# NCKempke/PIPS-IPMpp

Measured on AMD Instinct MI355X. Metric: KKT factor+solve per IPM iter/sec, N-block arrowhead LP, higher is better.
Workload: dtype f64; 1 GPU; 64 blocks x 10000 vars (5000 eq rows, rho=0.001), Schur dim 2000, 64 blocks/GPU [BASELINE configs[1]]; deterministic=False, family=random, root=dense LDL^T, sparse_head=multifrontal (k_front), solves_per_unit=4, collective=none, nnzL_per_gpu=649118456

## Files before the change

### pips-ipmpp_amd/csrc/engine.hip

```cpp
#include <hip/hip_runtime.h>

#include <algorithm>
#include <cstdlib>
#include <cstring>
#include <map>
#include <memory>
#include <mutex>
#include <thread>
#include <vector>

#include "common.h"
#include "devmem.h"
#include "layout.h"
#include "kernels.hip.h"
#include "rootkernel.hip.h"
#include "tailkernel.hip.h"
#include "pips_hip.h"

namespace pips {

static thread_local std::string g_last_error;
void set_last_error(const std::string& msg) { g_last_error = msg; }
std::atomic<long long> g_host_waits{0};
struct WaitSite { std::atomic<const char*> file{nullptr}; std::atomic<int> line{0}; std::atomic<long long> n{0}; };
// ... 82 lines not shown
         end(upd_diag[j]);
         begin(upd[j]);
         const int P = (pair2 > 1 && panel == 0 && split_diag && diag_ahead) ? pair2 : 1;
         const int g = j / P * P, q = j - g;
         if (j > p0 && split_diag && diag_ahead)
            for (int b = 0; b < nblk; ++b)
               if (blks[b].ntc > j + 1) {
                  const int k0 = std::max(p0, fst(b, j + 1)), lo = q > 0 ? std::max(k0, g) : k0;
                  if (lo < j) all.push_back({b, j + 1, j + 1, lo | (j << 16)});
               }
         if (P > 1 && q == 0 && j > p0)
            for (int b = 0; b < nblk; ++b)
               for (int d = j + 2; d <= j + P && d < blks[b].ntc; ++d) {
                  const int k0 = std::max(p0, fst(b, d));
                  if (k0 < j) all.push_back({b, d, d, k0 | (j << 16)});
               }
         if (j > p0)
            for (int b = 0; b < nblk; ++b)
               if (blks[b].ntc > j)
                  for (int ti = split_diag ? j + 1 : j; ti < blks[b].ntr; ++ti) {
                     if (j >= fst(b, ti)) {
                        const int k0 = std::max({p0, fst(b, ti), fst(b, j)}), lo = q > 0 ? std::max(k0, g) : k0;
                        if (lo < j) all.push_back({b, ti, j, lo | (j << 16)});
                     }
                     if (P > 1 && q == 0)
                        for (int c = j + 1; c < j + P && c < blks[b].ntc && c < ti; ++c)
                           if (c >= fst(b, ti)) {
                              const int k0 = std::max({p0, fst(b, ti), fst(b, c)});
                              if (k0 < j) all.push_back({b, ti, c, k0 | (j << 16)});
                           }
                  }
         end(upd[j]);
         begin(diag[j]);
         for (int b = 0; b < nblk; ++b)
            if (blks[b].ntc > j) all.push_back({b, j, j, 0});
         end(diag[j]);
         begin(trsm[j]);
         for (int b = 0; b < nblk; ++b)
            if (blks[b].ntc > j)
               for (int ti = j + 1; ti < blks[b].ntr; ++ti)
                  if (j >= fst(b, ti)) all.push_back({b, ti, j, 0});
         end(trsm[j]);
         begin(fwd[j]);
         for (int b = 0; b < nblk; ++b)
            if (blks[b].ntc > j)
               for (int ti = j; ti < blks[b].ntc; ++ti)
                  if (ti == j || (j >= 1 && j - 1 >= fst(b, ti))) all.push_back({b, ti, j, 0});
         end(fwd[j]);
         begin(bwd[j]);
         for (int b = 0; b < nblk; ++b)
            if (blks[b].ntc > j)
               for (int tj = 0; tj <= j; ++tj)
                  if (tj == j || (j + 1 < blks[b].ntc && tj >= fst(b, j + 1))) all.push_back({b, tj, j, 0});
         end(bwd[j]);
         if (panel > 0 && (j + 1) % panel == 0) {
            begin(trail_next[j]);
            if (lookahead)
               for (int b = 0; b < nblk; ++b)
                  if (j + 1 < blks[b].ntc)
                     for (int ti = j + 1; ti < blks[b].ntr; ++ti) all.push_back({b, ti, j + 1, p0 | ((j + 1) << 16)});
            end(trail_next[j]);
            begin(trail[j]);
            for (int b = 0; b < nblk; ++b)
               for (int tj = j + (lookahead ? 2 : 1); tj < blks[b].ntc; ++tj)
                  for (int ti = tj; ti < blks[b].ntr; ++ti) all.push_back({b, ti, tj, p0 | ((j + 1) << 16)});
            end(trail[j]);
         }
      }
      begin(schur);
      for (int b = 0; b < nblk; ++b)
         if (blks[b].ntc > 0 && blks[b].nb > 0) {
            const int nt = blks[b].nb_pad / TILE;
            for (int ti = 0; ti < nt; ++ti)
               for (int tj = 0; tj <= ti; ++tj) all.push_back({b, ti, tj, 0});
         }
      end(schur);
      h_tasks = all;
      return d_tasks.upload(all);
   }
};

struct SweepRt {
   DevBuf<TileTask> d_tasks;
   int n_tasks = 0;
   DevBuf<int> d_ints;
   long long n_flags = 0;
   DevBuf<long long> d_flag_off, d_tfirst_off;
   DevBuf<int> d_tfirst;
   int epoch = 0;
   bool enabled = false;
   long long poll_limit = SWEEP_POLL_LIMIT;
   int take_error(const char* who) {
      if (!d_ints) return PIPS_OK;
      int w = 0;
      HIP_TRY(hipMemcpy(&w, d_ints + 2 * SWEEP_NRHS_MAX, sizeof(int), hipMemcpyDeviceToHost));
      if (!w) return PIPS_OK;
      HIP_TRY(hipMemset(d_ints + 2 * SWEEP_NRHS_MAX, 0, sizeof(int)));
      PIPS_FAIL(PIPS_ERR_HIP, "%s: a single-launch solve sweep gave up waiting for a piece of the solution after %lld polls (its output is NaN); "
                              "another process holding the device for seconds can cause that - PIPS_HIP_SWEEP_LAUNCHES=1 selects the launch-per-column sweeps",
                who, poll_limit);
   }
   int build(const std::vector<BlkDesc>& blks, const std::vector<const std::vector<int>*>* first) {
      *this = SweepRt();
      if (const char* pl = getenv("PIPS_HIP_SWEEP_POLL_LIMIT")) poll_limit = atoll(pl);
      const int nblk = (int)blks.size();
      int ntc_max = 0;
      for (auto& b : blks) ntc_max = std::max(ntc_max, b.ntc);
      std::vector<TileTask> tasks;
      for (int i = 0; i < ntc_max; ++i)
         for (int b = 0; b < nblk; ++b)
            if (i < blks[b].ntc) tasks.push_back({b, i, 0, 0});
      n_tasks = (int)tasks.size();
      std::vector<long long> foff(nblk), tfoff(nblk);
      std::vector<int> tf;
      long long nf = 0;
      for (int b = 0; b < nblk; ++b) {
         foff[b] = nf;
         nf += blks[b].ntc;
         tfoff[b] = (long long)tf.size();
         if (first)
            for (int i = 0; i < blks[b].ntr; ++i) tf.push_back(i < blks[b].ntc ? std::min(i, (*(*first)[b])[i]) : (*(*first)[b])[i]);
      }
      int rc;
      if ((rc = d_tasks.upload(tasks))) return rc;
      if ((rc = d_flag_off.upload(foff))) return rc;
      if (first) {
         if ((rc = d_tfirst.upload(tf))) return rc;
         if ((rc = d_tfirst_off.upload(tfoff))) return rc;
      }
      n_flags = std::max<long long>(nf, 1);
      const size_t ints = (size_t)(2 * SWEEP_NRHS_MAX + 2 + n_flags * SWEEP_NRHS_MAX);
      PIPS_TRY(d_ints.alloc_zero(ints));
      epoch = 0;
      enabled = n_tasks > 0 && !getenv("PIPS_HIP_SWEEP_LAUNCHES");
      return PIPS_OK;
   }
   SweepArgs args(long long xw_stride, hipStream_t st) {
      int* ep = d_ints + 2 * SWEEP_NRHS_MAX + 1;
      hipLaunchKernelGGL(k_sweep_bump, dim3(1), dim3(1), 0, st, ep);
      return SweepArgs{d_tasks, n_tasks, d_ints, d_ints + 2 * SWEEP_NRHS_MAX + 2, d_flag_off, d_tfirst, d_tfirst_off, ep,
                       d_ints + 2 * SWEEP_NRHS_MAX, n_flags, xw_stride, poll_limit};
   }
};

struct PhaseTimer {
   bool on = false;
   struct Rec { hipEvent_t a, b; int phase; };
   std::vector<Rec> recs;
   std::vector<hipEvent_t> pool;
   size_t used = 0;
   static constexpr int NPHASE = 16;
   double ms[NPHASE] = {0};
   long long cnt[NPHASE] = {0};
   hipEvent_t get() {
      if (used == pool.size()) {
         hipEvent_t e;
         (void)hipEventCreate(&e);
         pool.push_back(e);
      }
      return pool[used++];
   }
   void reset() { recs.clear(); used = 0; }
   void begin(hipStream_t s, int phase) {
      if (!on) return;
      Rec r{get(), get(), phase};
      (void)hipEventRecord(r.a, s);
      recs.push_back(r);
   }
   void end(hipStream_t s) {
      if (!on) return;
      (void)hipEventRecord(recs.back().b, s);
   }
   int begin_i(hipStream_t s, int phase) {
      if (!on) return -1;
      begin(s, phase);
      return (int)recs.size() - 1;
   }
   void end_i(int idx, hipStream_t s) {
      if (on && idx >= 0) (void)hipEventRecord(recs[idx].b, s);
   }
   void collect() {
      for (int i = 0; i < NPHASE; ++i) { ms[i] = 0; cnt[i] = 0; }
      for (auto& r : recs) {
         float t = 0;
         if (hipEventElapsedTime(&t, r.a, r.b) == hipSuccess) { ms[r.phase] += t; ++cnt[r.phase]; }
      }
   }
   ~PhaseTimer() { for (auto e : pool) (void)hipEventDestroy(e); }
};

struct TailSingle {
   TailLdlArgs args{};
   DevBuf<TileTask> d_tasks;
   DevBuf<int> d_flags, d_flags_init, d_ctl;
   DevBuf<long long> d_flag_off;
   long long n_flags = 0;
   int n_tasks = 0, n_blocks = 0;
   int build(const TailPlan& p, const std::vector<BlkDesc>& blks, hipStream_t stream) {
      *this = TailSingle();
      const int nblk = (int)blks.size();
      n_blocks = nblk;
      std::vector<long long> foff(nblk + 1, 0);
      for (int b = 0; b < nblk; ++b) foff[b + 1] = foff[b] + (long long)blks[b].ntr * blks[b].ntc + blks[b].ntr + blks[b].ntc;
      n_flags = foff[nblk];
      std::vector<int> init((size_t)std::max<long long>(n_flags, 1), 0);
      for (int b = 0; b < nblk; ++b)
         for (int ti = 0; ti < blks[b].ntr; ++ti)
            for (int tj = 0; tj < blks[b].ntc; ++tj) init[foff[b] + (long long)ti * blks[b].ntc + tj] = -1;
      std::vector<TileTask> order;
      auto take = [&](const TaskList& l, int kind) {
         for (long long q = l.off; q < l.off + l.cnt; ++q) {
            TileTask t = p.h_tasks[q];
            if (t.blk < 0) continue;
            if (kind == ROOT_UPD) {
               int& pr = init[foff[t.blk] + (long long)t.ti * blks[t.blk].ntc + t.tj];
               if (pr < 0) pr = t.pad & 0xffff;
            } else
               t.pad = 0;
            t.blk |= kind << 24;
            order.push_back(t);
         }
      };
      std::vector<int> row_first((size_t)std::max<long long>(n_flags, 1), 1 << 20);
// ... 171 lines not shown
         hipLaunchKernelGGL(k_tile_diag, dim3(p.diag[j].cnt), dim3(256), 0, c.side, p.d_tasks + p.diag[j].off,
                            c.d_blks, c.d_arena, c.d_dtail, c.d_winv, c.d_psign, c.d_psign_off, c.d_inertia, c.d_pref);
         HIP_TRY(hipEventRecord(c.ev_rest, c.side));
      } else if (p.upd_diag[j].cnt > 0) {
         gemm_diag_tiles(p.upd_diag[j], c.stream);
      }
      if (p.upd[j].cnt > 0) {
         if (c.timer) c.timer->begin(c.stream, 2);
         gemm0(p.upd[j], c.stream);
         if (c.timer) c.timer->end(c.stream);
      }
      if (ahead) {
         HIP_TRY(hipStreamWaitEvent(c.stream, c.ev_rest, 0));
      } else {
         if (c.timer) c.timer->begin(c.stream, 3);
         if (c.bunch_kaufman)
            hipLaunchKernelGGL(k_tile_diag_bk, dim3(p.diag[j].cnt), dim3(256), 0, c.stream, p.d_tasks + p.diag[j].off, c.d_blks, c.d_arena, c.d_dtail,
                               c.d_winv, c.d_inertia, c.d_pert_cnt, c.d_pert_list, c.bk_orig, c.bk_orig_ld, c.bk_orig_rowmajor, c.d_bk_perm, c.bk_isolate);
         else
         hipLaunchKernelGGL(k_tile_diag, dim3(p.diag[j].cnt), dim3(256), 0, c.stream, p.d_tasks + p.diag[j].off,
                            c.d_blks, c.d_arena, c.d_dtail, c.d_winv, c.d_psign, c.d_psign_off, c.d_inertia, c.d_pref);
         if (c.timer) c.timer->end(c.stream);
      }
      if (p.trsm[j].cnt > 0) {
         if (c.timer) c.timer->begin(c.stream, 4);
         hipLaunchKernelGGL(k_tile_gemm<1>, dim3((p.trsm[j].cnt + 7) / 8 * 8), dim3(512), 0, c.stream, p.d_tasks + p.trsm[j].off, p.trsm[j].cnt,
                            c.d_blks, c.d_arena, c.d_dtail, c.d_winv, c.d_bmap, (double*)nullptr, 0, (const int*)nullptr, c.d_uarena);
         if (c.timer) c.timer->end(c.stream);
         if (c.bunch_kaufman && c.is_root && c.d_pert_cnt)
            hipLaunchKernelGGL(k_bk_growth, dim3(TILE), dim3(256), 0, c.stream, c.d_blks, c.d_arena, j, 1e8, c.d_pert_cnt, c.d_pert_list);
      }
      if (p.trail_next[j].cnt > 0 || p.trail[j].cnt > 0) {
         if ((rc = main_writes(j + 1))) return rc;
         const bool split = c.side && p.trail[j].cnt > 0;
         if (split) {
            HIP_TRY(hipEventRecord(c.ev_panel, c.stream));
            HIP_TRY(hipStreamWaitEvent(c.side, c.ev_panel, 0));
            gemm0(p.trail[j], c.side);
            HIP_TRY(hipEventRecord(c.ev_rest, c.side));
            side_busy = true;
            side_from = j + 2;
         }
         if (c.timer) c.timer->begin(c.stream, 2);
         if (p.trail_next[j].cnt > 0) gemm0(p.trail_next[j], c.stream);
         if (!split && p.trail[j].cnt > 0) gemm0(p.trail[j], c.stream);
         if (c.timer) c.timer->end(c.stream);
      }
   }
   if ((rc = main_writes(1 << 30))) return rc;
   if (SC && c.det_rounds) {
      if (c.timer) c.timer->begin(c.stream, 5);
      for (const TaskList& l : *c.det_rounds)
         if (l.cnt > 0)
            hipLaunchKernelGGL(k_tile_gemm<2>, dim3((l.cnt + 7) / 8 * 8), dim3(512), 0, c.stream, c.d_det_tasks + l.off, l.cnt, c.d_blks, c.d_arena,
                               c.d_dtail, c.d_winv, c.d_bmap, SC, ldSC, c.d_sctab, c.d_uarena, c.d_gbuf, c.gstride, c.d_blk_group);
      if (!c.det_reduce_later) reduce_det_groups(c, SC, ldSC);
      if (c.timer) c.timer->end(c.stream);
   } else if (SC && c.sc_groups && !c.d_sctab) {
      if (c.timer) c.timer->begin(c.stream, 5);
      for (size_t g = 0; g < c.sc_groups->size(); ++g) {
         const TaskList& l = (*c.sc_groups)[g];
         if (l.cnt > 0)
            hipLaunchKernelGGL(k_tile_gemm<2>, dim3((l.cnt + 7) / 8 * 8), dim3(512), 0, c.stream, c.d_sc_tasks + l.off, l.cnt, c.d_blks, c.d_arena,
                               c.d_dtail, c.d_winv, c.d_bmap, SC, ldSC, c.d_sctab, c.d_uarena);
         HIP_TRY(hipEventRecord((*c.ev_sc)[g], c.stream));
      }
      if (c.timer) c.timer->end(c.stream);
   } else if (SC && p.schur.cnt > 0 && c.d_ctr_pool && !c.d_sctab && *c.ctr_cursor < GEMM_CTR_SLOTS) {
      if (c.timer) c.timer->begin(c.stream, 5);
      const int wgs = ((p.schur.cnt + 7) / 8 * 8) / 8 * 9;
      hipLaunchKernelGGL(k_tile_gemm_bal<2>, dim3((wgs + 7) / 8 * 8), dim3(512), 0, c.stream, p.d_tasks + p.schur.off, p.schur.cnt, c.d_blks,
                         c.d_arena, c.d_dtail, c.d_winv, c.d_bmap, SC, ldSC, c.d_sctab, c.d_uarena, c.d_ctr_pool + 8 * (*c.ctr_cursor)++);
      if (c.timer) c.timer->end(c.stream);
   } else if (SC && p.schur.cnt > 0) {
      if (c.timer) c.timer->begin(c.stream, 5);
      hipLaunchKernelGGL(k_tile_gemm<2>, dim3((p.schur.cnt + 7) / 8 * 8), dim3(512), 0, c.stream, p.d_tasks + p.schur.off, p.schur.cnt, c.d_blks,
                         c.d_arena, c.d_dtail, c.d_winv, c.d_bmap, SC, ldSC, c.d_sctab, c.d_uarena);
      if (c.timer) c.timer->end(c.stream);
   }
   HIP_TRY(hipGetLastError());
   return PIPS_OK;
}

static int tail_fwd(const TailCtx& c, double* xw, int nrhs = 1, long long xw_stride = 0) {
   const TailPlan& p = *c.plan;
   if (c.sweep && c.sweep->enabled && nrhs <= SWEEP_NRHS_MAX) {
      hipLaunchKernelGGL(k_tail_rows_fwd, dim3(c.sweep->n_tasks, nrhs), dim3(256), 0, c.stream, c.sweep->args(xw_stride, c.stream), c.d_blks, c.d_arena, c.d_dtail,
                         c.d_winv, xw);
      HIP_TRY(hipGetLastError());
      return PIPS_OK;
   }
   for (int j = 0; j < p.ntc_max; ++j)
      if (p.fwd[j].cnt > 0)
         hipLaunchKernelGGL(k_tail_fwd, dim3(p.fwd[j].cnt, nrhs), dim3(256), 0, c.stream, p.d_tasks + p.fwd[j].off, c.d_blks,
                            c.d_arena, c.d_dtail, c.d_winv, xw, j, xw_stride);
   HIP_TRY(hipGetLastError());
   return PIPS_OK;
}

static int tail_bwd(const TailCtx& c, double* xw, int nrhs = 1, long long xw_stride = 0, int border = 0) {
   const TailPlan& p = *c.plan;
   if (p.ntc_max == 0) return PIPS_OK;
   if (border && !(c.sweep && c.sweep->enabled)) PIPS_FAIL(PIPS_ERR_STATE, "border-backward sweep needs the single-launch tail sweeps");
   if (c.sweep && c.sweep->enabled && nrhs <= SWEEP_NRHS_MAX) {
      hipLaunchKernelGGL(k_tail_rows_bwd, dim3(c.sweep->n_tasks, nrhs), dim3(256), 0, c.stream, c.sweep->args(xw_stride, c.stream), c.d_blks, c.d_arena, c.d_dtail,
                         c.d_winv, xw, border);
      HIP_TRY(hipGetLastError());
      return PIPS_OK;
   }
   for (int i = p.ntc_max - 1; i >= 0; --i)
      if (p.bwd[i].cnt > 0)
         hipLaunchKernelGGL(k_tail_bwd, dim3(p.bwd[i].cnt, nrhs), dim3(256), 0, c.stream, p.d_tasks + p.bwd[i].off, c.d_blks,
                            c.d_arena, c.d_dtail, c.d_winv, xw, i, xw_stride);
   HIP_TRY(hipGetLastError());
   return PIPS_OK;
}


struct AnalyzeKnobs : LayoutKnobs {
   long long tail_poll_limit = 0;
   int tail_diag_blocked = 1;
};
struct Engine;
static void read_layout_knobs(const Engine* e, AnalyzeOptions& opt, AnalyzeKnobs& knobs);

struct EngineAnalysis {
   DevBuf<double> d_norms;
   PinnedBuf<double> h_norms;
   DevBuf<int> d_frowptr, d_fcol, d_fsrc;
   DevBuf<long long> d_flong;
   DevBuf<int> d_sctab;
   DevBuf<int> d_schur_cols, d_schur_slot;
   DevBuf<int> d_kb_rec;
   DevBuf<long long> d_kb_off;
   DevBuf<int> d_kb_list;
   DevBuf<int> d_kb_tail;
   DevBuf<double> d_mfU;
   DevBuf<double> d_mfLV;
   DevBuf<int> d_roots, d_root_off;
   DevBuf<BbBatch> d_bb_batches;
   DevBuf<BbMeta> d_bb_meta;
   DevBuf<int> d_bb_off, d_bb_pos;
   DevBuf<double> d_bb_out;
   DevBuf<int> d_bb_round_blk;
   DevBuf<int> d_round_blk;
   DevBuf<int> d_mfint;
   DevBuf<long long> d_mfdbg;
   DevBuf<int> d_spine, d_spine_off;
   TailPlan plan;
   SweepRt sweep;
   TailSingle tsingle;
   DevBuf<double> d_uarena;
   DevBuf<double> d_arena, d_kval, d_bval, d_winv, d_dtail, d_xw, d_rhs, d_res, d_stage, d_pref;
   DevBuf<long long> d_kdst, d_bdst, d_kdiag, d_kptr, d_psign_off, d_perm_off, d_rowbase, d_bt_xoff;
   DevBuf<SnDesc> d_sns;
   DevBuf<BlkDesc> d_blks;
   DevBuf<int> d_lf_rows, d_lf_ptr, d_lf_src, d_lf_pos;
   DevBuf<double> d_lf_val;
   DevBuf<LeafDesc> d_leafdesc;
   DevBuf<int> d_lb_list;
   DevBuf<int> d_rowidx, d_upd, d_sncol, d_bmap, d_perm, d_inertia, d_nprimal;
   DevBuf<int> d_br_rowptr, d_br_sc, d_br_src;
   DevBuf<int> d_krowptr, d_kcolidx, d_bt_rowptr, d_bt_colidx, d_bt_rowsc;
   DevBuf<signed char> d_psign;
   struct GatherList {
      long long n_targets = 0, n_slots = 0;
      DevBuf<long long> d_tgt, d_off, d_slots;
   };
   struct SlotEntry { long long target, slot; };
   DevBuf<double> d_slot_val, d_vslot_val;
// ... 1141 lines not shown
      const bool need_amax = refine_mode == 1 && h_amax.empty();
      if (need_amax) {
         tmp.resize(nblk);
         HIP_TRY(hipMemcpyAsync(tmp.data(), d_blks, (size_t)nblk * sizeof(BlkDesc), hipMemcpyDeviceToHost, stream));
      }
      HIP_TRY(hipStreamSynchronize(stream));
      if (need_amax) {
         h_amax.resize(nblk);
         for (int b = 0; b < nblk; ++b) h_amax[b] = tmp[b].repl_abs / (repl_rel > 0 ? repl_rel : 1.0);
      }
      double worst = 0.0;
      for (int b = 0; b < nblk; ++b) {
         const double den = refine_mode == 1 ? h_amax[b] * h_norms[2 * nblk + b] + h_norms[nblk + b] : h_norms[nblk + b];
         if (den > 0.0) { const double q = h_norms[b] / den; if (!(q <= worst)) worst = q; }
      }
      *worst_out = worst;
      last_refine_measure = worst;
      return PIPS_OK;
   }

   int fetch_inertia() {
      if (inertia_in_flight && h_inertia_pin) {
         HIP_TRY(hipEventSynchronize(ev_inertia));
         std::copy(h_inertia_pin.get(), h_inertia_pin + h_inertia.size(), h_inertia.begin());
         inertia_in_flight = false;
         inertia_on_host = true;
         if (tail_single && h_inertia_pin[3 * nblk]) {
            h_inertia_pin[3 * nblk] = 0;
            int fi[6] = {0, 0, 0, 0, 0, 0};
            (void)hipMemcpy(fi, tsingle.d_ctl + 10, sizeof(fi), hipMemcpyDeviceToHost);
            HIP_TRY(hipMemsetAsync(tsingle.d_ctl + 9, 0, 7 * sizeof(int), stream));
            PIPS_FAIL(PIPS_ERR_HIP, "the single-launch factorisation of the dense tails (PIPS_HIP_TAIL_SINGLE) gave up waiting for a tile after %lld polls - first: task "
                                    "kind %d on tile (%d, %d) of block %d; its factors are unusable.  Another process holding the device for seconds can cause that",
                      tsingle.args.poll_limit, fi[1], fi[2], fi[3], fi[5] - 1);
         }
         return PIPS_OK;
      }
      if (inertia_on_host) return PIPS_OK;
      HIP_TRY(hipMemcpyAsync(h_inertia.data(), d_inertia, h_inertia.size() * sizeof(int), hipMemcpyDeviceToHost, stream));
      HIP_TRY(hipStreamSynchronize(stream));
      return PIPS_OK;
   }

   long long aug_passes = 0;
   int perturbed_cache = -1;
   int perturbed_leaf_pivots(int* out) {
      if (perturbed_cache < 0) {
         int rc = fetch_inertia();
         if (rc) return rc;
         int z = 0;
         for (int b = 0; b < nblk; ++b) z += h_inertia[3 * b + 2];
         perturbed_cache = z;
      }
      *out = perturbed_cache;
      return PIPS_OK;
   }
   int forward_augmented(const double* b_dev, double* red) {
      if (!factored) PIPS_FAIL(PIPS_ERR_STATE, "solve called before factor");
      HIP_TRY(hipSetDevice(device));
      timer.begin(stream, 7);
      hipLaunchKernelGGL(k_border_fill, dim3(8, nblk), dim3(256), 0, stream, d_blks, d_bmap, (const double*)nullptr, d_xw, 0.0);
      hipLaunchKernelGGL(k_permute_in, dim3(64, nblk, 1), dim3(256), 0, stream, d_blks, d_perm, d_perm_off, b_dev, 0LL, d_xw, 0LL);
      timer.end(stream);
      timer.begin(stream, 8);
      for (const LevelRange& L : levels) {
         if (L.simple_cnt > 0 && lf_rows > 0)
            hipLaunchKernelGGL(k_leaf_fwd_gather, dim3((unsigned)((lf_rows + 255) / 256), 1), dim3(256), 0, stream, d_lf_rows, d_lf_ptr, d_lf_src, d_lf_val, d_xw,
                               0LL, (int)lf_rows);
         else if (L.simple_cnt > 0)
            hipLaunchKernelGGL(k_head_solve_simple, dim3((L.simple_cnt + 255) / 256, 1), dim3(256), 0, stream, d_sns, L.simple_begin, L.simple_cnt, d_blks,
                               d_rowidx, d_arena, d_xw, 0LL, 0);
         if (L.simple_cnt > 0 && n_lb > 0)
            hipLaunchKernelGGL(k_leaf_border, dim3((n_lb + 255) / 256), dim3(256), 0, stream, d_lb_list, n_lb, d_sns, d_blks, d_rowidx, d_arena, d_xw, 0);
         const int begin = L.small_cnt > 0 ? L.small_begin : L.large_begin;
         const int cnt = L.small_cnt + L.large_cnt;
         if (cnt > 0)
            hipLaunchKernelGGL(head_wcap <= 16 ? k_head_fwd_chain<16> : k_head_fwd_chain<HEAD_WMAX>, dim3(cnt, 1), dim3(64), 0, stream, d_sns, begin, d_blks,
                               d_rowidx, d_arena, d_xw, 0LL, 1);
      }
      timer.end(stream);
      timer.begin(stream, 9);
      TailCtx c = ctx();
      c.timer = nullptr;
      int rc = tail_fwd(c, d_xw);
      if (rc) return rc;
      if (nb_pad_max > 0)
         hipLaunchKernelGGL(k_tail_border_fwd, dim3(nb_pad_max / TILE, nblk), dim3(256), 0, stream, d_blks, d_arena, d_dtail, d_xw);
      hipLaunchKernelGGL(k_border_collect, dim3(8, nblk), dim3(256), 0, stream, d_blks, d_bmap, d_xw, red);
      timer.end(stream);
      ++aug_passes;
      HIP_TRY(hipGetLastError());
      return PIPS_OK;
   }
   int forward_augmented_det(const double* b_dev) {
      if (!factored) PIPS_FAIL(PIPS_ERR_STATE, "solve called before factor");
      if (!det_aug_ready || !head_slots) PIPS_FAIL(PIPS_ERR_STATE, "forward_augmented_det: not prepared");
      HIP_TRY(hipSetDevice(device));
      timer.begin(stream, 7);
      hipLaunchKernelGGL(k_border_fill, dim3(8, nblk), dim3(256), 0, stream, d_blks, d_bmap, (const double*)nullptr, d_xw, 0.0);
      hipLaunchKernelGGL(k_permute_in, dim3(64, nblk, 1), dim3(256), 0, stream, d_blks, d_perm, d_perm_off, b_dev, 0LL, d_xw, 0LL);
      timer.end(stream);
      timer.begin(stream, 8);
      const ScatterCtx sxv{2, nullptr, d_vslot_val, d_xw, nullptr};
      for (size_t li = 0; li < levels.size(); ++li) {
         const LevelRange& L = levels[li];
         gather(gv_levels[li], d_vslot_val, d_xw);
         if (L.simple_cnt > 0 && lf_rows > 0)
            hipLaunchKernelGGL(k_leaf_fwd_gather, dim3((unsigned)((lf_rows + 255) / 256), 1), dim3(256), 0, stream, d_lf_rows, d_lf_ptr, d_lf_src, d_lf_val, d_xw,
                               0LL, (int)lf_rows);
         else if (L.simple_cnt > 0)
            hipLaunchKernelGGL(k_head_solve_simple, dim3((L.simple_cnt + 255) / 256, 1), dim3(256), 0, stream, d_sns, L.simple_begin, L.simple_cnt, d_blks,
                               d_rowidx, d_arena, d_xw, 0LL, 0, sxv);
         const int begin = L.small_cnt > 0 ? L.small_begin : L.large_begin;
         const int cnt = L.small_cnt + L.large_cnt;
         if (cnt > 0) hipLaunchKernelGGL(k_head_fwd, dim3(cnt, 1), dim3(64), 0, stream, d_sns, begin, d_blks, d_rowidx, d_arena, d_xw, 0LL, sxv);
      }
      gather(gv_tail, d_vslot_val, d_xw);
      hipLaunchKernelGGL(k_border_rowdot_det, dim3(grid_for(n_bg_ent, 256, 1 << 20)), dim3(256), 0, stream, n_bg_ent, d_bg_ent, d_arena, d_xw, d_bg_val);
      hipLaunchKernelGGL(k_border_gather_det, dim3((unsigned)((n_bg_targets + 3) / 4)), dim3(256), 0, stream, n_bg_targets, d_bg_ptr, d_bg_idx, d_bg_slot, d_bg_val, d_xw);
      timer.end(stream);
      timer.begin(stream, 9);
      TailCtx c = ctx();
      c.timer = nullptr;
      int rc = tail_fwd(c, d_xw);
      if (rc) return rc;
      if (nb_pad_max > 0)
         hipLaunchKernelGGL(k_tail_border_fwd, dim3(nb_pad_max / TILE, nblk), dim3(256), 0, stream, d_blks, d_arena, d_dtail, d_xw);
      timer.end(stream);
      ++aug_passes;
      HIP_TRY(hipGetLastError());
      return PIPS_OK;
   }
   int backward_augmented(const double* x0_dev, double* out_dev) {
      if (!factored) PIPS_FAIL(PIPS_ERR_STATE, "solve called before factor");
      HIP_TRY(hipSetDevice(device));
      timer.begin(stream, 10);
      hipLaunchKernelGGL(k_border_fill, dim3(8, nblk), dim3(256), 0, stream, d_blks, d_bmap, x0_dev, d_xw, 1.0);
      TailCtx c = ctx();
      c.timer = nullptr;
      int rc = tail_bwd(c, d_xw, 1, 0, 1);
      if (rc) return rc;
      for (int l = (int)levels.size() - 1; l >= 0; --l) {
         const LevelRange& L = levels[l];
         const int begin = L.small_cnt > 0 ? L.small_begin : L.large_begin;
         const int cnt = L.small_cnt + L.large_cnt;
         if (cnt > 0)
            hipLaunchKernelGGL(head_wcap <= 16 ? k_head_bwd_chain<16> : k_head_bwd_chain<HEAD_WMAX>, dim3(cnt, 1), dim3(64), 0, stream, d_sns, begin, d_blks,
                               d_rowidx, d_arena, d_xw, 0LL, 1, 1);
         if (L.simple_cnt > 0 && d_leafdesc)
            hipLaunchKernelGGL(k_leaf_bwd, dim3((L.simple_cnt + 255) / 256, 1), dim3(256), 0, stream, d_leafdesc, L.simple_cnt, d_rowidx, d_arena, d_xw, 0LL, 1);
         else if (L.simple_cnt > 0)
            hipLaunchKernelGGL(k_head_solve_simple, dim3((L.simple_cnt + 255) / 256, 1), dim3(256), 0, stream, d_sns, L.simple_begin, L.simple_cnt, d_blks,
                               d_rowidx, d_arena, d_xw, 0LL, 1, sx_atomic(), 0, 0, 1);
         if (L.simple_cnt > 0 && n_lb > 0)
            hipLaunchKernelGGL(k_leaf_border, dim3((n_lb + 255) / 256), dim3(256), 0, stream, d_lb_list, n_lb, d_sns, d_blks, d_rowidx, d_arena, d_xw, 1);
      }
      timer.end(stream);
      timer.begin(stream, 7);
      hipLaunchKernelGGL(k_permute_out, dim3(64, nblk, 1), dim3(256), 0, stream, d_blks, d_perm, d_perm_off, out_dev, 0LL, d_xw, 0LL);
      timer.end(stream);
      HIP_TRY(hipGetLastError());
      return PIPS_OK;
   }
   int solve_border_backward(const double* x0_dev, double* out_dev) {
      if (!factored) PIPS_FAIL(PIPS_ERR_STATE, "solve called before factor");
      HIP_TRY(hipSetDevice(device));
      HIP_TRY(hipMemsetAsync(d_xw, 0, (size_t)xw_total * sizeof(double), stream));
      hipLaunchKernelGGL(k_border_fill, dim3(8, nblk), dim3(256), 0, stream, d_blks, d_bmap, x0_dev, d_xw);
      TailCtx c = ctx();
      int rc = tail_bwd(c, d_xw, 1, 0, 1);
      if (rc) return rc;
      const ScatterCtx none{0, nullptr, nullptr, nullptr, nullptr};
      if (spine_total > 0)
         hipLaunchKernelGGL(k_head_solve_spine, dim3(nblk, 1), dim3(64), 0, stream, d_spine, d_spine_off, d_sns, d_blks, d_rowidx, d_arena, d_xw, 0LL, 1, 1);
      for (int l = (int)levels.size() - 1; l >= 0; --l) {
         const LevelRange& L = levels[l];
         const int begin = L.small_cnt > 0 ? L.small_begin : L.large_begin;
         const int cnt = L.small_cnt + L.large_cnt;
         if (cnt > 0)
            hipLaunchKernelGGL(head_wcap <= 16 ? k_head_bwd_chain<16> : k_head_bwd_chain<HEAD_WMAX>, dim3(cnt, 1), dim3(64), 0, stream, d_sns, begin,
                               d_blks, d_rowidx, d_arena, d_xw, 0LL, 1, 0);
         if (L.simple_cnt > 0)
            hipLaunchKernelGGL(k_head_solve_simple, dim3((L.simple_cnt + 255) / 256, 1), dim3(256), 0, stream, d_sns, L.simple_begin, L.simple_cnt,
                               d_blks, d_rowidx, d_arena, d_xw, 0LL, 1, none, 1);
      }
      hipLaunchKernelGGL(k_permute_out, dim3(64, nblk, 1), dim3(256), 0, stream, d_blks, d_perm, d_perm_off, out_dev, 0LL, d_xw, 0LL);
      HIP_TRY(hipGetLastError());
      return PIPS_OK;
   }
};

static void read_layout_knobs(const Engine* e, AnalyzeOptions& opt, AnalyzeKnobs& knobs) {
   opt.tile = TILE;
   opt.max_sn_width = 16;
   if (const char* sw = getenv("PIPS_HIP_SN_WIDTH")) opt.max_sn_width = std::max(1, std::min(HEAD_WMAX, atoi(sw)));
   else if (e && e->sn_width > 0) opt.max_sn_width = std::min(HEAD_WMAX, e->sn_width);
   if (const char* rz = getenv("PIPS_HIP_RELAX_ZEROS")) opt.relax_zeros = atof(rz);
   if (const char* ndd = getenv("PIPS_HIP_ND_DEPTH")) opt.nd_depth = atoi(ndd);
   if (const char* ndm = getenv("PIPS_HIP_ND_MIN")) opt.nd_min_size = atoi(ndm);
   if (const char* ml = getenv("PIPS_HIP_MF_LDS")) opt.mf_lds_doubles = atoll(ml);
   if (const char* sp = getenv("PIPS_HIP_MF_SPLIT")) opt.mf_split_nb_max = atoi(sp) == 0 ? 0 : std::min(176, std::max(atoi(sp), 2));
   knobs.deterministic = e && e->deterministic;
   knobs.schur_mode = e ? e->schur_mode : 0;
   knobs.mf_lds_doubles = opt.mf_lds_doubles;
   knobs.mf_wanted = env_int("PIPS_HIP_MF", 1) != 0;
   if (!knobs.mf_wanted) opt.mf_split_nb_max = 0;
   opt.mf_konly = opt.mf_split_nb_max > 0 && !knobs.deterministic && opt.max_sn_width <= 16 && env_int("PIPS_HIP_MF_KONLY", 0) != 0;
   knobs.spine = env_flag("PIPS_HIP_SPINE");
   knobs.tail_single = env_flag("PIPS_HIP_TAIL_SINGLE");
// ... 1703 lines not shown
```

### pips-ipmpp_amd/csrc/kernels.hip.h

```cpp
#pragma once
#include <hip/hip_runtime.h>
#include <stdint.h>

#include "records.h"

namespace pips {

constexpr int KB = 16;
constexpr int LDS_PAD = 16;
constexpr int LDSW = TILE + LDS_PAD;

typedef double double4_t __attribute__((ext_vector_type(4)));

struct BelowRow { const double* p; long long stride; };
__device__ __forceinline__ BelowRow below_row(const double* __restrict__ arena, const SnDesc& sn, int a) {
   if (a < sn.ld - sn.w) return BelowRow{arena + sn.panel + sn.w + a, (long long)sn.ld};
   return BelowRow{arena + sn.bb + (a - sn.rb), (long long)((sn.r - sn.rb + 3) & ~3)};
}

__device__ __forceinline__ void atomic_add_f64(double* p, double v) {
   __hip_atomic_fetch_add(p, v, __ATOMIC_RELAXED, __HIP_MEMORY_SCOPE_AGENT);
}

struct ScatterCtx {
// ... 2126 lines not shown
   const int tid = threadIdx.x, tj = task.ti, ld = bd.ldT;
   double* xt = xw + bd.xw_off + bd.n_head;
   const bool upd = i + 1 < bd.ntc;
   double vnext = 0.0, dsc = 0.0;
   if (upd && tid < TILE) vnext = xt[(i + 1) * TILE + tid];
   double acc = tid < TILE ? xt[tj * TILE + tid] : 0.0;
   if (tj == i && tid < TILE) dsc = dtail[bd.dt_off + i * TILE + tid];
   tg_d2 m[32];
   if (upd) tile_tload(m, arena + bd.T + (long long)(i + 1) * TILE + (long long)tj * TILE * ld, ld, tid);
   const double* Wi = winv + bd.winv_off + (long long)i * TILE * TILE;
   if (upd) {
      if (tid < TILE) v[tid] = vnext;
      __syncthreads();
      tile_tdot(m, v, outp, tid);
      __syncthreads();
      if (tid < TILE) acc -= outp[tid];
   }
   if (tj == i) {
      __syncthreads();
      if (tid < TILE) v[tid] = acc * dsc;
      __syncthreads();
      tile_tload(m, Wi, TILE, tid);
      tile_tdot(m, v, outp, tid);
      __syncthreads();
      if (tid < TILE) acc = outp[tid];
   }
   if (tid < TILE) xt[tj * TILE + tid] = acc;
}

struct SweepArgs {
   const TileTask* tasks;
   int n_tasks;
   int* ticket;
   int* flags;
   const long long* flag_off;
   const int* tfirst;
   const long long* tfirst_off;
   const int* epoch_ptr;
   int* err;
   long long flag_stride, xw_stride;
   long long poll_limit;
};
constexpr long long SWEEP_POLL_LIMIT = 4000000;
constexpr int SWEEP_NRHS_MAX = 32;

__global__ void k_sweep_bump(int* epoch) { *epoch += 1; }

__device__ __forceinline__ bool sweep_wait(const int* f, int epoch, long long poll_limit = SWEEP_POLL_LIMIT) {
   long long spins = 0;
   while (__hip_atomic_load(f, __ATOMIC_RELAXED, __HIP_MEMORY_SCOPE_AGENT) != epoch) {
      __builtin_amdgcn_s_sleep(4);
      if (++spins > poll_limit) return false;
   }
   return true;
}
__device__ __forceinline__ int sweep_ticket(const SweepArgs& a, int* sh) {
   if (threadIdx.x == 0) *sh = __hip_atomic_fetch_add(a.ticket + 2 * blockIdx.y, 1, __ATOMIC_RELAXED, __HIP_MEMORY_SCOPE_AGENT);
   __syncthreads();
   return *sh;
}
__device__ __forceinline__ void sweep_done(const SweepArgs& a) {
   if (threadIdx.x == 0) {
      int* t = a.ticket + 2 * blockIdx.y;
      const int d = __hip_atomic_fetch_add(t + 1, 1, __ATOMIC_RELAXED, __HIP_MEMORY_SCOPE_AGENT);
      if (d == a.n_tasks - 1) {
         __hip_atomic_store(t, 0, __ATOMIC_RELAXED, __HIP_MEMORY_SCOPE_AGENT);
         __hip_atomic_store(t + 1, 0, __ATOMIC_RELAXED, __HIP_MEMORY_SCOPE_AGENT);
      }
   }
}
__device__ __forceinline__ double sweep_load(const double* p) {
   return __hip_atomic_load(p, __ATOMIC_RELAXED, __HIP_MEMORY_SCOPE_AGENT);
}
__device__ __forceinline__ void sweep_store(double* p, double x) {
   __hip_atomic_store(p, x, __ATOMIC_RELAXED, __HIP_MEMORY_SCOPE_AGENT);
}
__device__ __forceinline__ void sweep_publish(int* flag, int epoch) {
   asm volatile("s_waitcnt vmcnt(0)" ::: "memory");
   __syncthreads();
   if (threadIdx.x == 0) __hip_atomic_store(flag, epoch, __ATOMIC_RELAXED, __HIP_MEMORY_SCOPE_AGENT);
}
__device__ __forceinline__ double sweep_nan() { return __builtin_nan(""); }

__global__ __launch_bounds__(256) void k_tail_rows_fwd(SweepArgs a, const BlkDesc* __restrict__ blks, const double* __restrict__ arena,
                                                      const double* __restrict__ dtail, const double* __restrict__ winv,
                                                      double* __restrict__ xw) {
   __shared__ double v[TILE];
   __shared__ double part[TILE];
   __shared__ int sh_t, sh_ok;
   const int epoch = *a.epoch_ptr;
   const int t = sweep_ticket(a, &sh_t);
   const TileTask task = a.tasks[t];
   const BlkDesc bd = blks[task.blk];
   const int tid = threadIdx.x, row = tid & 127, half = tid >> 7, i = task.ti, ld = bd.ldT;
   double* xt = xw + a.xw_stride * blockIdx.y + bd.xw_off + bd.n_head;
   int* fl = a.flags + a.flag_stride * blockIdx.y + a.flag_off[task.blk];
   const int j0 = a.tfirst ? min(i, a.tfirst[a.tfirst_off[task.blk] + i]) : 0;
   const double* Lrow = arena + bd.T + (long long)i * TILE;
   double acc = half == 0 ? xt[i * TILE + row] : 0.0;
   double m[64];
   bool ok = true;
   if (j0 < i) {
      tile_load_half(m, Lrow + (long long)j0 * TILE * ld, ld, row, half);
      for (int j = j0;; ++j) {
         if (tid == 0) sh_ok = sweep_wait(fl + j, epoch, a.poll_limit) ? 1 : 0;
         __syncthreads();
         if (!sh_ok) { ok = false; break; }
         if (tid < TILE) v[tid] = sweep_load(xt + j * TILE + tid) * dtail[bd.dt_off + j * TILE + tid];
         __syncthreads();
         const double s = tile_dot_half(m, v, half);
         if (half == 1) part[row] = s;
         __syncthreads();
         if (half == 0) acc -= s + part[row];
         if (j + 1 >= i) break;
         __builtin_amdgcn_sched_barrier(0);
         tile_load_half(m, Lrow + (long long)(j + 1) * TILE * ld, ld, row, half);
      }
   }
   if (ok) {
      __syncthreads();
      if (half == 0) v[row] = acc;
      __syncthreads();
      __builtin_amdgcn_sched_barrier(0);
      tile_load_half(m, winv + bd.winv_off + (long long)i * TILE * TILE, TILE, row, half);
      const double s = tile_dot_half(m, v, half);
      if (half == 1) part[row] = s;
      __syncthreads();
      if (half == 0) acc = s + part[row];
   } else {
      acc = sweep_nan();
      if (tid == 0) *a.err = 1;
   }
   if (half == 0) sweep_store(xt + i * TILE + row, acc);
   sweep_publish(fl + i, epoch);
   sweep_done(a);
}

__global__ __launch_bounds__(256) void k_tail_rows_bwd(SweepArgs a, const BlkDesc* __restrict__ blks, const double* __restrict__ arena,
                                                      const double* __restrict__ dtail, const double* __restrict__ winv,
                                                      double* __restrict__ xw, int border = 0) {
   __shared__ double v[TILE];
   __shared__ double outp[TILE];
   __shared__ int sh_t, sh_ok;
   const int epoch = *a.epoch_ptr;
   const int t = sweep_ticket(a, &sh_t);
   const TileTask task = a.tasks[a.n_tasks - 1 - t];
   const BlkDesc bd = blks[task.blk];
   const int tid = threadIdx.x, i = task.ti, ld = bd.ldT;
   double* xt = xw + a.xw_stride * blockIdx.y + bd.xw_off + bd.n_head;
   int* fl = a.flags + a.flag_stride * blockIdx.y + a.flag_off[task.blk];
   const int* tf = a.tfirst ? a.tfirst + a.tfirst_off[task.blk] : nullptr;
   const double* Lcol = arena + bd.T + (long long)i * TILE * ld;
   auto next_k = [&](int k) {
      while (k > i && tf && tf[k] > i) --k;
      return k;
   };
   double acc = tid < TILE ? xt[i * TILE + tid] : 0.0;
   const double dsc = tid < TILE ? dtail[bd.dt_off + i * TILE + tid] : 0.0;
   tg_d2 m[32];
   int k = next_k((border ? bd.ntr : bd.ntc) - 1);
   bool ok = true;
   if (k > i) {
      tile_tload(m, Lcol + (long long)k * TILE, ld, tid);
      for (;;) {
         if (k < bd.ntc) {
            if (tid == 0) sh_ok = sweep_wait(fl + k, epoch, a.poll_limit) ? 1 : 0;
            __syncthreads();
            if (!sh_ok) { ok = false; break; }
            if (tid < TILE) v[tid] = sweep_load(xt + k * TILE + tid);
         } else {
            __syncthreads();
            if (tid < TILE) v[tid] = xt[k * TILE + tid];
         }
         __syncthreads();
         tile_tdot(m, v, outp, tid);
         __syncthreads();
// ... 868 lines not shown
```

Before: 8.278 64-block work units/s (1 factorize + 4 solveCompressed).

## Fold border-row forward updates into the single-launch tail forward sweep

Appends border-row tile tasks to the persistent forward sweep task list. Each border task waits on the per-column flags and accumulates its update as soon as each tail column is published, so no separate k_tail_border_fwd launch has to wait for the whole sweep to finish. The intent is to overlap the border work with the triangular sweep and drop one kernel launch per solve pass. In exchange, border tasks occupy workgroups that spin-wait on flags, and an env knob can switch back to the separate launch.

```diff
diff --git a/pips-ipmpp_amd/csrc/engine.hip b/pips-ipmpp_amd/csrc/engine.hip
--- a/pips-ipmpp_amd/csrc/engine.hip
+++ b/pips-ipmpp_amd/csrc/engine.hip
@@ -188,7 +188,8 @@
 
 struct SweepRt {
    DevBuf<TileTask> d_tasks;
-   int n_tasks = 0;
+   int n_tasks = 0, n_fwd_tasks = 0;
+   bool fwd_border = false;
    DevBuf<int> d_ints;
    long long n_flags = 0;
    DevBuf<long long> d_flag_off, d_tfirst_off;
@@ -217,6 +218,10 @@
          for (int b = 0; b < nblk; ++b)
             if (i < blks[b].ntc) tasks.push_back({b, i, 0, 0});
       n_tasks = (int)tasks.size();
+      for (int b = 0; b < nblk; ++b)
+         if (blks[b].m > 0 && blks[b].nb > 0)
+            for (int ib = 0; ib < blks[b].nb_pad / TILE; ++ib) tasks.push_back({b, blks[b].ntc + ib, 0, 0});
+      n_fwd_tasks = (int)tasks.size();
       std::vector<long long> foff(nblk), tfoff(nblk);
       std::vector<int> tf;
       long long nf = 0;
@@ -239,12 +244,13 @@
       PIPS_TRY(d_ints.alloc_zero(ints));
       epoch = 0;
       enabled = n_tasks > 0 && !getenv("PIPS_HIP_SWEEP_LAUNCHES");
-      return PIPS_OK;
-   }
-   SweepArgs args(long long xw_stride, hipStream_t st) {
+      fwd_border = enabled && n_fwd_tasks > n_tasks && env_int("PIPS_HIP_AUG_FWD_SPLIT", 0) == 0;
+      return PIPS_OK;
+   }
+   SweepArgs args(long long xw_stride, hipStream_t st, int n = -1) {
       int* ep = d_ints + 2 * SWEEP_NRHS_MAX + 1;
       hipLaunchKernelGGL(k_sweep_bump, dim3(1), dim3(1), 0, st, ep);
-      return SweepArgs{d_tasks, n_tasks, d_ints, d_ints + 2 * SWEEP_NRHS_MAX + 2, d_flag_off, d_tfirst, d_tfirst_off, ep,
+      return SweepArgs{d_tasks, n < 0 ? n_tasks : n, d_ints, d_ints + 2 * SWEEP_NRHS_MAX + 2, d_flag_off, d_tfirst, d_tfirst_off, ep,
                        d_ints + 2 * SWEEP_NRHS_MAX, n_flags, xw_stride, poll_limit};
    }
 };
@@ -582,10 +588,12 @@
    return PIPS_OK;
 }
 
-static int tail_fwd(const TailCtx& c, double* xw, int nrhs = 1, long long xw_stride = 0) {
+static int tail_fwd(const TailCtx& c, double* xw, int nrhs = 1, long long xw_stride = 0, int border = 0) {
    const TailPlan& p = *c.plan;
+   if (border && !(c.sweep && c.sweep->fwd_border && nrhs == 1)) PIPS_FAIL(PIPS_ERR_STATE, "forward sweep with border rows needs the single-launch tail sweeps");
    if (c.sweep && c.sweep->enabled && nrhs <= SWEEP_NRHS_MAX) {
-      hipLaunchKernelGGL(k_tail_rows_fwd, dim3(c.sweep->n_tasks, nrhs), dim3(256), 0, c.stream, c.sweep->args(xw_stride, c.stream), c.d_blks, c.d_arena, c.d_dtail,
+      const int n = border ? c.sweep->n_fwd_tasks : c.sweep->n_tasks;
+      hipLaunchKernelGGL(k_tail_rows_fwd, dim3(n, nrhs), dim3(256), 0, c.stream, c.sweep->args(xw_stride, c.stream, n), c.d_blks, c.d_arena, c.d_dtail,
                          c.d_winv, xw);
       HIP_TRY(hipGetLastError());
       return PIPS_OK;
@@ -1893,9 +1901,9 @@
       timer.begin(stream, 9);
       TailCtx c = ctx();
       c.timer = nullptr;
-      int rc = tail_fwd(c, d_xw);
+      int rc = tail_fwd(c, d_xw, 1, 0, sweep.fwd_border);
       if (rc) return rc;
-      if (nb_pad_max > 0)
+      if (nb_pad_max > 0 && !sweep.fwd_border)
          hipLaunchKernelGGL(k_tail_border_fwd, dim3(nb_pad_max / TILE, nblk), dim3(256), 0, stream, d_blks, d_arena, d_dtail, d_xw);
       hipLaunchKernelGGL(k_border_collect, dim3(8, nblk), dim3(256), 0, stream, d_blks, d_bmap, d_xw, red);
       timer.end(stream);
@@ -1933,9 +1941,9 @@
       timer.begin(stream, 9);
       TailCtx c = ctx();
       c.timer = nullptr;
-      int rc = tail_fwd(c, d_xw);
+      int rc = tail_fwd(c, d_xw, 1, 0, sweep.fwd_border);
       if (rc) return rc;
-      if (nb_pad_max > 0)
+      if (nb_pad_max > 0 && !sweep.fwd_border)
          hipLaunchKernelGGL(k_tail_border_fwd, dim3(nb_pad_max / TILE, nblk), dim3(256), 0, stream, d_blks, d_arena, d_dtail, d_xw);
       timer.end(stream);
       ++aug_passes;
diff --git a/pips-ipmpp_amd/csrc/kernels.hip.h b/pips-ipmpp_amd/csrc/kernels.hip.h
--- a/pips-ipmpp_amd/csrc/kernels.hip.h
+++ b/pips-ipmpp_amd/csrc/kernels.hip.h
@@ -2232,6 +2232,41 @@
 }
 __device__ __forceinline__ double sweep_nan() { return __builtin_nan(""); }
 
+__device__ __forceinline__ void sweep_fwd_border(const SweepArgs& a, const BlkDesc& bd, int blk, int i, int epoch, const double* __restrict__ arena,
+                                                 const double* __restrict__ dtail, double* __restrict__ xw, double* v, double* part, int* sh_ok) {
+   const int tid = threadIdx.x, row = tid & 127, half = tid >> 7, ld = bd.ldT, ntc = bd.ntc;
+   double* xt = xw + a.xw_stride * blockIdx.y + bd.xw_off + bd.n_head;
+   const int* fl = a.flags + a.flag_stride * blockIdx.y + a.flag_off[blk];
+   const int j0 = a.tfirst ? min(ntc, a.tfirst[a.tfirst_off[blk] + i]) : 0;
+   const double* Lrow = arena + bd.T + (long long)i * TILE;
+   double acc = 0.0;
+   double m[64];
+   bool ok = true;
+   if (j0 < ntc) {
+      tile_load_half(m, Lrow + (long long)j0 * TILE * ld, ld, row, half);
+      for (int j = j0;; ++j) {
+         if (tid == 0) *sh_ok = sweep_wait(fl + j, epoch, a.poll_limit) ? 1 : 0;
+         __syncthreads();
+         if (!*sh_ok) { ok = false; break; }
+         if (tid < TILE) v[tid] = sweep_load(xt + j * TILE + tid) * dtail[bd.dt_off + j * TILE + tid];
+         __syncthreads();
+#pragma unroll
+         for (int c = 0; c < 64; ++c) acc += m[c] * v[half * 64 + c];
+         asm volatile("" : "+v"(acc));
+         if (j + 1 >= ntc) break;
+         __builtin_amdgcn_sched_barrier(0);
+         tile_load_half(m, Lrow + (long long)(j + 1) * TILE * ld, ld, row, half);
+      }
+   }
+   if (!ok && tid == 0) *a.err = 1;
+   if (half == 1) part[row] = acc;
+   __syncthreads();
+   if (half == 0) {
+      double* xb = xt + i * TILE + row;
+      *xb = ok ? *xb - (acc + part[row]) : sweep_nan();
+   }
+}
+
 __global__ __launch_bounds__(256) void k_tail_rows_fwd(SweepArgs a, const BlkDesc* __restrict__ blks, const double* __restrict__ arena,
                                                       const double* __restrict__ dtail, const double* __restrict__ winv,
                                                       double* __restrict__ xw) {
@@ -2242,6 +2277,11 @@
    const int t = sweep_ticket(a, &sh_t);
    const TileTask task = a.tasks[t];
    const BlkDesc bd = blks[task.blk];
+   if (task.ti >= bd.ntc) {
+      sweep_fwd_border(a, bd, task.blk, task.ti, epoch, arena, dtail, xw, v, part, &sh_ok);
+      sweep_done(a);
+      return;
+   }
    const int tid = threadIdx.x, row = tid & 127, half = tid >> 7, i = task.ti, ld = bd.ldT;
    double* xt = xw + a.xw_stride * blockIdx.y + bd.xw_off + bd.n_head;
    int* fl = a.flags + a.flag_stride * blockIdx.y + a.flag_off[task.blk];
```

Result: no change. 8.304 64-block work units/s (1 factorize + 4 solveCompressed), median of 6 (+0.3%).
